# alberto-paparella/MusicRecommendation

Hardware: AMD Instinct MI355X
Metric: scored (test-user,song) pairs/sec, ItemBasedModel, 1/2/4/8 MI355X + mAP@10 (higher is better)
Workload: dtype int64

## Files before the change

### include/mr_engine.h

```cpp
#ifndef MR_ENGINE_H
#define MR_ENGINE_H

#include <stdint.h>
#include <stddef.h>

#ifdef __cplusplus
extern "C" {
#endif

#define MR_OK          0
#define MR_E_INVALID  -1
#define MR_E_HIP      -2
#define MR_E_OOM      -3
#define MR_E_STATE    -4
#define MR_E_IO       -5
#define MR_E_PARSE    -6
#define MR_E_RCCL     -7

#define MR_UBM 0
#define MR_IBM 1

#define MR_OUT_F32 0
#define MR_OUT_F64 1

// ... 42 lines not shown

int mr_launch_info(const mr_ctx* ctx, int32_t* shape, int32_t* block_songs, int32_t* n_tiles);

int mr_batch_info(const mr_ctx* ctx, int32_t* batch, int32_t* chunk, int32_t* n_chunks);

int mr_route_info(const mr_ctx* ctx, int32_t* route, int32_t* n_rows, int64_t* pool_entries);

int mr_topk_mode(const mr_ctx* ctx, int32_t* candidate_only);

int mr_cooc_stats(mr_ctx* ctx, int64_t* index_nnz, int64_t* consumed, int64_t* build_reads);

typedef struct mr_cooc_bytes_t {
  int64_t heavy_rows, light_rows;
  int64_t heavy_reads, light_reads;
  int64_t heavy_index_bytes, light_index_bytes;
  int64_t heavy_visits;
  int64_t consumed_bytes;
  int64_t group_tiles;
  int64_t n_groups;
  int64_t index_sparse_entries, index_dense_songs;
  int64_t consumed_sparse_entries, consumed_dense_songs;
} mr_cooc_bytes_t;
int mr_cooc_bytes(mr_ctx* ctx, mr_cooc_bytes_t* out);

int mr_shard_tile_songs(const mr_options* opt, int32_t n_train_users, int32_t n_test_users,
                        int32_t* tile_songs);

int mr_shard_tile_songs_n(const mr_options* opt, int32_t n_train_users, int32_t n_test_users, int32_t n_songs,
                          int32_t n_shards, int32_t* tile_songs);

int mr_run(mr_ctx* ctx, int model);
int mr_sync(mr_ctx* ctx);

int mr_graph_capture(mr_ctx* ctx, int model, int32_t n_steps);
int mr_graph_launch(mr_ctx* ctx);

int mr_device_outputs(const mr_ctx* ctx, void** dense, int32_t** topk_songs,
                      int64_t** topk_keys, double** topk_scores);

int mr_run_into(mr_ctx* ctx, int model, void* dense_dev);

typedef struct mr_view {
  int32_t n_test_users, n_songs, song_lo, song_hi, out_dtype, device;
  const int64_t* te_off;
  const int32_t* te_songs;
  void* stream;
// ... 134 lines not shown
```

### musicrecommendation_amd/_lib.py

```python
from __future__ import annotations

import ctypes
import os
from ctypes import POINTER, c_char_p, c_double, c_int, c_int32, c_int64, c_void_p

_HERE = os.path.dirname(os.path.abspath(__file__))
_VARIANT = os.environ.get("MR_ENGINE_LIB", "")
LIB_PATH = os.path.join(_HERE, f"libmr_engine_{_VARIANT}.so" if _VARIANT else "libmr_engine.so")

MR_OK = 0
MR_E_INVALID = -1
MR_E_HIP = -2
MR_E_OOM = -3
MR_E_STATE = -4
MR_E_IO = -5
MR_E_PARSE = -6
MR_E_RCCL = -7
MR_TRANSPORT_AUTO, MR_TRANSPORT_COPY, MR_TRANSPORT_RCCL = 0, 1, 2
MR_UBM = 0
MR_IBM = 1
STAGE1 = {"auto": 0, "fused": 1, "separate": 2, "wide": 4}
SHAPES = {0: "separate", 1: "fused", 3: "wide"}
MR_OUT_F32 = 0
MR_OUT_F64 = 1
# ... 80 lines not shown
MR_COMB_AGGREGATION = 1
MR_COMB_STOCHASTIC = 2
MR_SWEEP_MAX_PARAMS = 64


class EngineError(RuntimeError):
    def __init__(self, code: int, where: str, msg: str):
        super().__init__(f"{where}: {_ERRNAMES.get(code, code)}: {msg}")
        self.code = code


SIGNATURES = {
    "mr_options_default": (c_int, [POINTER(MrOptions)]),
    "mr_create": (c_int, [POINTER(MrOptions), POINTER(c_void_p)]),
    "mr_destroy": (c_int, [c_void_p]),
    "mr_load": (c_int, [c_void_p, POINTER(MrDataset)]),
    "mr_shard_info": (c_int, [c_void_p, POINTER(c_int32), POINTER(c_int32), POINTER(c_int32)]),
    "mr_launch_info": (c_int, [c_void_p, POINTER(c_int32), POINTER(c_int32), POINTER(c_int32)]),
    "mr_batch_info": (c_int, [c_void_p, POINTER(c_int32), POINTER(c_int32), POINTER(c_int32)]),
    "mr_route_info": (c_int, [c_void_p, POINTER(c_int32), POINTER(c_int32), POINTER(c_int64)]),
    "mr_topk_mode": (c_int, [c_void_p, POINTER(c_int32)]),
    "mr_cooc_stats": (c_int, [c_void_p, POINTER(c_int64), POINTER(c_int64), POINTER(c_int64)]),
    "mr_cooc_bytes": (c_int, [c_void_p, POINTER(MrCoocBytes)]),
    "mr_shard_tile_songs": (c_int, [POINTER(MrOptions), c_int32, c_int32, POINTER(c_int32)]),
    "mr_shard_tile_songs_n": (c_int, [POINTER(MrOptions), c_int32, c_int32, c_int32, c_int32, POINTER(c_int32)]),
    "mr_run": (c_int, [c_void_p, c_int]),
    "mr_sync": (c_int, [c_void_p]),
    "mr_graph_capture": (c_int, [c_void_p, c_int, c_int32]),
    "mr_graph_launch": (c_int, [c_void_p]),
    "mr_device_outputs": (c_int, [c_void_p, POINTER(c_void_p), POINTER(c_void_p), POINTER(c_void_p), POINTER(c_void_p)]),
    "mr_score_dense": (c_int, [c_void_p, c_int, c_void_p]),
    "mr_topk": (c_int, [c_void_p, c_int, c_int, c_void_p, c_void_p, c_void_p]),
    "mr_copy_dense": (c_int, [c_void_p, c_void_p]),
    "mr_copy_topk": (c_int, [c_void_p, c_void_p, c_void_p, c_void_p]),
    "mr_copy_topk_device": (c_int, [c_void_p, c_void_p, c_void_p]),
    "mr_copy_topk_device_async": (c_int, [c_void_p, c_void_p, c_void_p]),
    "mr_topk_merge_device_async": (c_int, [c_void_p, c_int32, c_int32, c_int32, c_void_p, c_void_p, c_void_p, c_void_p,
                                           c_void_p]),
    "mr_topk_record_bytes": (c_int, [c_int32, c_int32, POINTER(c_int64)]),
    "mr_topk_merge_records_async": (c_int, [c_void_p, c_int32, c_int32, c_int32, c_void_p, c_int64, c_void_p, c_void_p,
                                            c_void_p]),
    "mr_topk_merge_host": (c_int, [c_int32, c_int32, c_int32, c_void_p, c_void_p, c_void_p, c_void_p, c_void_p, c_void_p]),
    "mr_topk_merge_device": (c_int, [c_void_p, c_int32, c_int32, c_int32, c_void_p, c_void_p, c_void_p, c_void_p, c_void_p, c_void_p]),
    "mr_kernel_times": (c_int, [c_void_p, c_int32, POINTER(c_int64), POINTER(c_double), c_int32]),
    "mr_debug_stamps": (c_int, [c_void_p, c_void_p, c_int64]),
    "mr_timing_begin": (c_int, [c_void_p]),
# ... 93 lines not shown
```

### musicrecommendation_amd/csrc/mr_engine.hip

```cpp
#include <hip/hip_runtime.h>

#include <algorithm>
#include <atomic>
#include <climits>
#include <cmath>
#include <cstdarg>
#include <cstdio>
#include <cstdlib>
#include <cstring>
#include <limits>
#include <mutex>
#include <string>
#include <vector>

#ifndef MR_TILE_ROWS
#define MR_TILE_ROWS 32
#endif

#include "mr_engine.h"
#include "mr_internal.h"
#include "mr_par.h"


namespace {
// ... 2656 lines not shown
      run += wave_lane(inc, 63);
    }
    if (lane == 0) p.row_nnz[r] = (unsigned)run;
  }
  wave_lds_sync();
  stamp_rt_wave(sb, 3);
  unsigned* out = p.pool + p.row_base[r];
  for (int i = lane; i < S; i += 64) {
    const unsigned x = tab[i];
    if (x) {
      const int key = (int)((x >> kLightCntBits) - 1u);
      const int t = tile_of(key, bs, inv_bs);
      const int pos = atomicAdd(&tpos[t], 1);
      out[pos] = ((unsigned)(key - t * bs) << kCoocCntBits) | (x & kLightCntMask);
    }
  }
  wave_lds_sync();
  stamp_rt_wave(sb, 4);
  stamp_val(sb, 5, n, true);
  stamp_val(sb, 6, S, true);
  stamp_val(sb, 7, 64, true);
}

constexpr int kMaxGroupTiles = 8;
__host__ __device__ inline int cooc_group_lds(int bs, int g) {
  return align16(g * bs * 2) + 3 * kMaxGroupTiles * 4 + kMaxGroupTiles * 16 * 4;
}

__device__ __forceinline__ unsigned nz_halves(unsigned x) {
  return (((x & 0x7fff7fffu) + 0x7fff7fffu) | x) & 0x80008000u;
}
__device__ __forceinline__ int nz_pairs8(const uint4& w) {
  return __popc(nz_halves(w.x) | (nz_halves(w.y) >> 1) | (nz_halves(w.z) >> 2) | (nz_halves(w.w) >> 3));
}

template <int NT>
__device__ __forceinline__ void cooc_emit_group16(const CoocParams& p, int r, bool big, int t0, int ntg, int bs,
                                                  int width, const unsigned* cnt, int* s_wcnt, int* s_tail,
                                                  long long* off, unsigned* row_nz, long long* sb = nullptr) {
  constexpr int NW = NT / 64;
  const int tid = threadIdx.x, lane = tid & 63, w = tid >> 6;
  for (int k = 0; k < ntg; ++k) {
    const int bw = min(width, (t0 + k + 1) * bs) - (t0 + k) * bs;
    const uint4* cv = reinterpret_cast<const uint4*>(cnt + (size_t)k * (bs >> 1));
    const int nch = (bw + 7) >> 3;
    int nz = 0;
// ... 325 lines not shown
int light_tier_go(hipStream_t st, int n, const CoocParams* lp) {
  constexpr int NT = light_tier_nt(T), S = light_tier_slots(T);
  const int lds = cooc_light_lds<NT, S>();
  if (!lp) {
    MR_HIP(hipFuncSetAttribute((const void*)k_cooc_light<NT, S>, hipFuncAttributeMaxDynamicSharedMemorySize, lds));
    return MR_OK;
  }
  hipLaunchKernelGGL((k_cooc_light<NT, S>), dim3(n), dim3(NT), (size_t)lds, st, *lp);
  MR_HIP(hipGetLastError());
  return MR_OK;
}
template <int SW>
int light_wave_go(hipStream_t st, int n, const CoocParams* lp) {
  const int lds = cooc_wave_bytes<SW>() * kWaveRowsPerBlock;
  if (!lp) {
    MR_HIP(hipFuncSetAttribute((const void*)k_cooc_light_wave<SW>, hipFuncAttributeMaxDynamicSharedMemorySize, lds));
    return MR_OK;
  }
  hipLaunchKernelGGL(k_cooc_light_wave<SW>, dim3((n + kWaveRowsPerBlock - 1) / kWaveRowsPerBlock),
                     dim3(64 * kWaveRowsPerBlock), (size_t)lds, st, *lp, n);
  MR_HIP(hipGetLastError());
  return MR_OK;
}
int light_tier_call(int t, hipStream_t st, int n, const CoocParams* lp, const CoocParams&) {
  switch (t) {
    case 0: return light_tier_go<0>(st, n, lp);
    case 1: return light_tier_go<1>(st, n, lp);
    case 2: return light_tier_go<2>(st, n, lp);
    case 3: return light_tier_go<3>(st, n, lp);
    case 4: return light_wave_go<2048>(st, n, lp);
    default: return light_wave_go<1024>(st, n, lp);
  }
}

struct DenseTopkParams {
  int user0, width, song_lo, k;
  const void* dense;
  long long* top_key;
  int* top_song;
  double* top_score;
  unsigned* neg;
};

template <typename OutT>
__global__ __launch_bounds__(kWideThreads) void k_topk_dense(DenseTopkParams p) {
  constexpr int NT = kWideThreads, NW = NT / 64;
// ... 128 lines not shown
int dev_upload(DevBuf<T>& b, const T* src, size_t n, hipStream_t st) {
  int rc = dev_alloc(b, n);
  if (rc) return rc;
  if (n) MR_HIP(hipMemcpyAsync(b.p, src, n * sizeof(T), hipMemcpyHostToDevice, st));
  return MR_OK;
}

using ScoreKernel = void (*)(ScoreParams);
using NbrKernel = void (*)(NbrParams);

enum Shape { kShapeSeparate = 0, kShapeFused = 1, kShapeWide = 3 };

struct CoocPlan {
  int route = 1;
  std::vector<int32_t> row_song, te_row;
  std::vector<int64_t> row_base;
  std::vector<int64_t> row_reads;
  std::vector<int32_t> row_slots;
  std::vector<int32_t> heavy_rows, light_rows;
  std::vector<int32_t> shard_deg;
  std::vector<int32_t> row_users;
  std::vector<int32_t> row_listeners;
  std::vector<uint8_t> row_light;
  int64_t build_reads = 0;
  int64_t pool_cap = 0;
  int32_t max_shard_deg = 0;
  int n_light_tier[6] = {0, 0, 0, 0, 0, 0};
  bool all32 = false;
  int n_heavy32 = 0;
  int n_big16 = 0, tcap16 = 0, tcap32 = 0;
  int dense_div = 0, force32 = 0;
  unsigned sat = 255;
  int grp = 0, n_grp = 0, urec_words = 0, lrec_words = 0;
  int64_t n_lrec = 0;
  int64_t n_llrec = 0;
  int group_nt = 1024;
  int cooc_nt = 1024;
  int n_rows() const { return (int)row_song.size(); }
  int n_heavy() const { return (int)heavy_rows.size(); }
  int n_light() const { return (int)light_rows.size(); }
};

inline bool is_u32_row(const CoocPlan& p, int32_t listeners) { return p.all32 || listeners >= 65536; }

}

struct mr_ctx {
  mr_options opt{};
  int dev_share = 1;
  hipStream_t stream = nullptr;
  bool loaded = false;
  bool ran = false;
  bool fused = false;
  int shape = kShapeSeparate;
  int last_model = -1;
  int n_tr = 0, n_te = 0, n_s = 0;
  int song_lo = 0, song_hi = 0, width = 0;
  int block_songs = 0, n_tiles = 0;
  int cap = 0, batch = 0;
  int chunk = 1, n_chunks = 1;
  size_t score_lds = 0, nbr_lds = 0, merge_lds = 0, wide_lds = 0;
  ScoreKernel score_kernel[2] = {nullptr, nullptr};
  NbrKernel nbr_kernel[2] = {nullptr, nullptr};
// ... 30 lines not shown
  int graph_steps = 0;
  DevBuf<unsigned> flag;
  long long win_launches = 0;
  CoocPlan cooc;
  size_t cooc_score_lds = 0, cooc_lds = 0;
  int nseg = 0;
  ScoreKernel cooc_kernel = nullptr;
  DevBuf<int> row_song, te_row, seg_len;
  DevBuf<long long> row_base, seg_off;
  DevBuf<unsigned> pool;
  DevBuf<unsigned> row_nnz;
  bool cooc_ran = false;
  hipStream_t side[2] = {nullptr, nullptr};
  hipEvent_t side_fork = nullptr, side_join[2] = {nullptr, nullptr};
  size_t bstamp_off = 0;
  size_t lstamp_off = 0;
  DevBuf<int> rows_order, row_slots;
  DevBuf<int4> rdesc;
  DevBuf<long long> sr_off;
  DevBuf<unsigned> sr_songs;
  DevBuf<unsigned> urec;
  DevBuf<unsigned> lrec;
  DevBuf<uint2> llrec;

  void release_data() {
    tr_off.release(); te_off.release(); trs_off.release(); q_song.release();
    cand_key.release(); top_key.release(); nbr_q.release();
    tsongs.release(); tpack.release(); te_rng.release(); te_q.release(); te_sched.release(); sched_off.release(); te_songs.release(); trs_users.release(); toff.release(); sbound.release();
    nbr_v.release(); nbr_cnt.release(); cand_song.release(); top_song.release();
    counter.release();
    sqrt_c.release(); sqrt_tr.release(); sqrt_te.release(); top_score.release();
    rsq_c.release(); cand_on = false;
    dense.release();
    mm_key.release(); mm_on = mm_valid = false;
    stamps.release();
    flag.release();
    row_song.release(); te_row.release(); seg_len.release(); row_base.release(); seg_off.release();
    pool.release();
    rows_order.release(); row_slots.release(); sr_off.release(); sr_songs.release(); row_nnz.release();
    urec.release(); lrec.release(); llrec.release(); rdesc.release();
    cooc = CoocPlan{};
    cooc_kernel = nullptr;
    if (graph_exec) (void)hipGraphExecDestroy(graph_exec);
    if (graph) (void)hipGraphDestroy(graph);
    graph_exec = nullptr;
    graph = nullptr;
    graph_steps = 0;
    loaded = ran = cooc_ran = false;
// ... 59 lines not shown
    const int r = e ? std::atoi(e) : 32;
    return (r == 16 || r == 64) ? r : 32;
  }();
  return rows;
}

constexpr int64_t kLightSlotsNarrow = 8192;
int64_t cooc_light_max_opt(bool narrow) {
  const char* e = std::getenv("MR_COOC_LIGHT_MAX");
  int64_t v = e ? std::atoll(e) : (narrow ? kLightSlotsNarrow : kLightSlots);
  int64_t s = 1024;
  while (s * 2 <= std::min<int64_t>(v, kLightSlots)) s *= 2;
  return s;
}
int64_t cooc_light_load_opt() {
  const char* e = std::getenv("MR_COOC_LIGHT_LOAD");
  const int64_t v = e ? std::atoll(e) : 80;
  return std::min<int64_t>(100, std::max<int64_t>(10, v));
}
bool cooc_light_opt() {
  const char* e = std::getenv("MR_COOC_LIGHT");
  return !(e && std::atoi(e) == 0);
}
bool fused_sched_opt() {
  const char* e = std::getenv("MR_FUSED_SCHED");
  return MR_FUSED_SCHED && !(e && std::atoi(e) == 0);
}
int cooc_nt_opt() {
  const char* e = std::getenv("MR_COOC_NT");
  return e && std::atoi(e) == 512 ? 512 : 1024;
}
int cooc_group_nt_opt() {
  const char* e = std::getenv("MR_COOC_GNT");
  return e && std::atoi(e) == 512 ? 512 : 1024;
}
int cooc_group_max_opt() {
  const char* e = std::getenv("MR_COOC_GRP");
  const int v = e ? std::atoi(e) : 0;
  return v > 0 ? v : kMaxGroupTiles;
}
bool cooc_group_opt() {
  const char* e = std::getenv("MR_COOC_GROUP");
  return !(e && std::atoi(e) == 0);
}
bool cooc_side_opt() {
  const char* e = std::getenv("MR_COOC_SIDE");
  return !(e && std::atoi(e) == 0);
}
int cooc_dense_div_opt() {
  const char* e = std::getenv("MR_COOC_DENSE_DIV");
  return e ? std::max(0, std::atoi(e)) : kCoocDenseDiv;
}
int cooc_dense32_opt() {
  const char* e = std::getenv("MR_COOC_DENSE32");
  return e && std::atoi(e) == 1 ? 1 : 0;
}
unsigned cooc_sat_opt() {
  const char* e = std::getenv("MR_COOC_SAT");
  const long v = e ? std::atol(e) : 255;
  return (unsigned)std::min<long>(255, std::max<long>(1, v));
}

bool cooc_pays(double v_est, double e_est, const std::vector<int64_t>& bound, const std::vector<int64_t>& reads,
               const std::vector<int32_t>& row_song, const std::vector<int32_t>& col_tr, int n_tiles) {
  double build = 0.0;
  for (size_t r = 0; r < row_song.size(); ++r) {
    const double c = col_tr[row_song[r]];
    if (bound[r] <= light_bound_max(kLightSlots) && c <= kLightCntMask) build += 12.8e-12 * (double)(reads[r] - c) + 28e-9;
    else build += n_tiles * (35e-12 * c + 24e-9);
  }
  return build + 0.49e-12 * e_est < 5.75e-12 * v_est;
}

int wide_map_opt() {
  static const int m = [] {
    const char* e = std::getenv("MR_WIDE_MAP");
    const int v = e ? std::atoi(e) : 0;
    return v >= 1 && v <= 3 ? v : kWideMapDefault;
  }();
  return m;
}

int auto_block_songs(int width, int n_te, bool fused, int k, int n_tr) {
  long long cover = ((long long)width + 255) / 256 * 256;
  if (!fused && n_tr > kMaxLdsTrainUsers && k <= kMaxTopkLarge)
    return (int)std::max<long long>(256, std::min<long long>(kMaxBlockSongs, cover));
  const long long cap = k > 0 ? kMaxTopkTile : (fused ? 8192 : kMaxBlockSongs);
  const long long target = fused ? 256 : 1024;
  long long want = ((long long)width * std::max(1, n_te) + target - 1) / target;
  long long bs = ((want + 255) / 256) * 256;
  bs = std::max<long long>(256, std::min<long long>(cap, bs));
  return (int)std::max<long long>(256, std::min(bs, cover));
// ... 387 lines not shown
      return "a cheaper estimate than the two-hop route (auto)";
  }
  return nullptr;
}

void cooc_split(const CoocIn& in, CoocPlan& p) {
  const std::vector<int32_t>& col_tr = in.col_tr;
  const int width = in.lp.width, n_tiles = in.lp.n_tiles, bs = in.lp.block_songs;
  const int64_t nr = p.n_rows();
  const bool light_ok = width <= kLightMaxWidth && n_tiles <= kLightMaxTiles && cooc_light_opt();
  bool narrow = false;
  if (cooc_group_opt() && 1 + (n_tiles + 2) / 2 <= 32 && p.max_shard_deg <= 65535 &&
      n_tiles <= std::min(kMaxGroupTiles, cooc_group_max_opt()))
    narrow = cooc_group_lds(bs, n_tiles) <= kLdsBytes;
  const int64_t lload = cooc_light_load_opt(), light_slots_max = cooc_light_max_opt(narrow);
  p.dense_div = cooc_dense_div_opt();
  int64_t dense_pad = 0;
  for (int t = 0; t < n_tiles; ++t) {
    const int bw = (int)(std::min<int64_t>(width, (int64_t)(t + 1) * bs) - (int64_t)t * bs);
    dense_pad += cooc_dense_words(bw) - (bw + 3) / 4;
  }
  dense_pad = (dense_pad + 3) & ~(int64_t)3;
  p.row_slots.assign((size_t)std::max<int64_t>(1, nr), 0);
  for (int64_t r = 0; r < nr; ++r) {
    const int64_t c = col_tr[p.row_song[r]];
    if (light_ok && p.row_base[r] * 100 <= light_slots_max * lload && c <= (int32_t)kLightCntMask) {
      int sl = 1024;
      while ((int64_t)sl * lload < p.row_base[r] * 100) sl <<= 1;
      p.row_slots[r] = sl | (walk_glog(c > 0 ? (p.row_reads[r] - c) / c : 0) << kLightGlogShift);
      p.light_rows.push_back((int32_t)r);
      p.row_base[r] = (p.row_base[r] + 3) & ~(int64_t)3;
    } else {
      const int64_t nz = p.row_base[r];
      const int64_t dn = std::max<int64_t>(1, std::min<int64_t>(p.dense_div, width)) * nz;
      p.row_base[r] = ((std::min<int64_t>(width, dn) + nz + 3) & ~(int64_t)3) + 8 * (int64_t)n_tiles + dense_pad;
      p.heavy_rows.push_back((int32_t)r);
    }
  }
  std::vector<int32_t>& heavy_rows = p.heavy_rows;
  p.force32 = cooc_dense32_opt();
  p.all32 = !MR_COOC_P16 || p.force32;
  std::stable_partition(heavy_rows.begin(), heavy_rows.end(),
                        [&](int32_t r) { return is_u32_row(p, col_tr[p.row_song[r]]); });
  for (int32_t r : heavy_rows) p.n_heavy32 += is_u32_row(p, col_tr[p.row_song[r]]) ? 1 : 0;
  const int sparse_max = p.dense_div > 0 ? (bs + p.dense_div - 1) / p.dense_div : bs;
  p.tcap32 = (std::max(sparse_max, cooc_dense_words(bs) + bs) + 7) & ~7;
  p.tcap16 = p.tcap32;
  for (size_t i = p.n_heavy32; i < heavy_rows.size(); ++i) {
    if (col_tr[p.row_song[heavy_rows[i]]] < kCoocBigRow) break;
// ... 20 lines not shown
      if ((int)i >= p.n_heavy32 + p.n_big16)
        while (glog > 0 && cr > (int64_t)(p.group_nt >> glog) * kGroupPipeR) --glog;
      p.row_slots[r] = glog << kLightGlogShift;
    }
  } else {
    p.urec_words = 0;
  }
  p.pool_cap = mr_par::exclusive_scan(p.row_base.data(), nr);
  p.row_base[nr] = p.pool_cap;
}

void cooc_records(const CoocIn& in, CoocPlan& p) {
  if (p.grp > 0) {
    for (size_t i = p.n_heavy32; i < p.heavy_rows.size(); ++i) p.n_lrec += in.col_tr[p.row_song[p.heavy_rows[i]]];
    p.lrec_words = 1;
    while (2 * (p.lrec_words - 1) < p.n_grp + 1) p.lrec_words <<= 1;
  }
  for (int32_t r : p.light_rows) p.n_llrec += in.col_tr[p.row_song[r]];
}

void cooc_finish(const CoocIn& in, CoocPlan& p) {
  const int n_tiles = in.lp.n_tiles;
  const auto tier = [&](int32_t r) { return light_tier(p.row_slots[r] & kLightSlotsMask, n_tiles); };
  std::stable_sort(p.light_rows.begin(), p.light_rows.end(), [&](int32_t x, int32_t y) { return tier(x) < tier(y); });
  for (int32_t r : p.light_rows) p.n_light_tier[tier(r)]++;
  const size_t nr = p.row_song.size();
  for (int64_t x : p.row_reads) p.build_reads += x;
  p.row_users.assign(nr, 0);
  for (size_t i = 0; i < (size_t)in.d->te_off[in.d->n_test_users]; ++i)
    if (p.te_row[i] >= 0) p.row_users[p.te_row[i]]++;
  p.row_listeners.resize(nr);
  for (size_t r = 0; r < nr; ++r) p.row_listeners[r] = in.col_tr[p.row_song[r]];
  p.row_light.assign(nr, 0);
  for (int32_t r : p.light_rows) p.row_light[r] = 1;
  p.sat = cooc_sat_opt();
  p.cooc_nt = cooc_nt_opt();
  p.route = 2;
}

int plan_cooc(const CoocIn& in, size_t free_b, int dev_share, CoocPlan* out, const char** why) {
  *out = CoocPlan{};
  *why = nullptr;
  if (!in.lp.wide()) *why = "the wide shape only";
  else if (in.lp.block_songs > kCoocMaxTile) *why = "song tiles <= 32768";
  if (in.opt.ibm_route == 1) return MR_OK;
  CoocPlan p;
  if (!*why) *why = cooc_rows(in, p);
  if (!*why) *why = cooc_bounds(in, p);
  if (!*why) {
    cooc_split(in, p);
    for (int64_t r = 0; r < p.n_rows(); ++r)
      if (p.row_base[r] & 3)
        return fail(MR_E_STATE, "co-listening index: row %lld starts at word %lld (not 16-B aligned)",
                    (long long)r, (long long)p.row_base[r]);
    cooc_records(in, p);
// ... 96 lines not shown
  if ((rc = dev_alloc(c->pool, (size_t)p.pool_cap))) return rc;
  const size_t n_heavy = p.heavy_rows.size();
  std::vector<int32_t> order(p.heavy_rows);
  order.insert(order.end(), p.light_rows.begin(), p.light_rows.end());
  if ((rc = dev_upload(c->rows_order, order.data(), order.size(), st))) return rc;
  {
    std::vector<int4> rd(std::max<size_t>(1, order.size()));
    int64_t at_lrec = 0, at_llrec = 0;
    for (size_t i = 0; i < order.size(); ++i) {
      const int32_t r = order[i], s2 = p.row_song[r];
      const int cnt = (int)(trs_off[s2 + 1] - trs_off[s2]);
      int z = (int)trs_off[s2];
      if (p.grp > 0 && (int)i >= p.n_heavy32 && i < n_heavy) {
        z = (int)at_lrec;
        at_lrec += cnt;
      } else if (i >= n_heavy) {
        z = (int)at_llrec;
        at_llrec += cnt;
      }
      rd[i] = make_int4(r, p.row_slots[r], z, cnt);
    }
    if ((rc = dev_upload(c->rdesc, rd.data(), rd.size(), st))) return rc;
    MR_HIP(hipStreamSynchronize(st));
  }
  if ((rc = dev_upload(c->row_slots, p.row_slots.data(), p.row_slots.size(), st))) return rc;
  if (p.light_rows.empty() && p.grp == 0) return MR_OK;
  std::vector<int64_t> so((size_t)n_tr + 1, 0);
  std::copy(p.shard_deg.begin(), p.shard_deg.begin() + n_tr, so.begin());
  so[n_tr] = mr_par::exclusive_scan(so.data(), (int64_t)n_tr);
  mr_par::buffer<uint32_t> ss((size_t)so[n_tr] + 4);
  std::fill(ss.begin() + so[n_tr], ss.end(), 0u);
  mr_par::parallel_for(n_tr, [&](int64_t a, int64_t b, int) {
    for (int64_t v = a; v < b; ++v) {
      const int32_t* r0 = std::lower_bound(ti.songs.data() + ti.off[v], ti.songs.data() + ti.off[v + 1], lo);
      for (int64_t i = 0; i < so[v + 1] - so[v]; ++i) ss[so[v] + i] = (uint32_t)(r0[i] - lo);
    }
  });
  if ((rc = dev_upload(c->sr_off, reinterpret_cast<const long long*>(so.data()), so.size(), st))) return rc;
  if ((rc = dev_upload(c->sr_songs, ss.data(), ss.size(), st))) return rc;
  if (!p.light_rows.empty()) {
    if ((rc = dev_alloc(c->llrec, (size_t)std::max<int64_t>(1, p.n_llrec)))) return rc;
    hipLaunchKernelGGL(k_llrec, dim3((unsigned)p.light_rows.size()), dim3(256), 0, st, c->rdesc.p + n_heavy,
                       c->row_song.p, c->trs_off.p, c->trs_users.p, c->sr_off.p, c->llrec.p);
    MR_HIP(hipGetLastError());
  }
  if (p.grp > 0) {
    if ((rc = dev_alloc(c->urec, (size_t)std::max(1, n_tr) * p.urec_words))) return rc;
    hipLaunchKernelGGL(k_urec, dim3((std::max(1, n_tr) + 255) / 256), dim3(256), 0, st, c->sr_off.p,
                       c->sr_songs.p, n_tr, n_tiles, lp.block_songs, p.urec_words, c->urec.p);
    MR_HIP(hipGetLastError());
    if ((rc = dev_alloc(c->lrec, (size_t)std::max<int64_t>(1, p.n_lrec) * p.lrec_words))) return rc;
    const int n16 = (int)n_heavy - p.n_heavy32;
    if (n16 > 0)
      hipLaunchKernelGGL(k_lrec, dim3(n16), dim3(256), 0, st, c->rdesc.p + p.n_heavy32, c->row_song.p,
                         c->trs_off.p, c->trs_users.p, c->urec.p, p.urec_words, n_tiles, p.grp, p.n_grp, p.lrec_words,
                         c->lrec.p);
    MR_HIP(hipGetLastError());
    MR_HIP(hipStreamSynchronize(st));
    c->urec.release();
  }
  MR_HIP(hipStreamSynchronize(st));
  return MR_OK;
}

int alloc_outputs(mr_ctx* c, const LaunchPlan& lp, int route, int n_te) {
  hipStream_t st = c->stream;
  const int k = lp.k;
// ... 48 lines not shown
    const WideLds<kWideThreads> WL = p.cooc_nt == 512 ? wide_lds<512>(bs, k, n_chunks).as_wide()
                                                      : wide_lds<kWideThreads>(bs, k, n_chunks);
    c->cooc_score_lds = (size_t)WL.total;
    c->nseg = std::min(std::min(p.cooc_nt, (WL.total - WL.wk - 8) / 40), 255);
    if (c->nseg < 16) return fail(MR_E_INVALID, "co-listening route: no LDS for row descriptors");
    c->cooc_lds = (size_t)cooc_build_lds<false>(bs);
    if (p.grp > 0)
      MR_HIP(hipFuncSetAttribute(p.group_nt == 512 ? (const void*)k_cooc_group<512> : (const void*)k_cooc_group<1024>,
                                 hipFuncAttributeMaxDynamicSharedMemorySize, cooc_group_lds(bs, p.grp)));
    for (int t = 0; t < kLightTiers; ++t)
      if (int rc2 = light_tier_call(t, nullptr, 0, nullptr, CoocParams{})) return rc2;
    MR_HIP(hipFuncSetAttribute((const void*)c->cooc_kernel, hipFuncAttributeMaxDynamicSharedMemorySize,
                               (int)c->cooc_score_lds));
    MR_HIP(hipFuncSetAttribute((const void*)k_cooc_build<MR_COOC_NT, false>, hipFuncAttributeMaxDynamicSharedMemorySize,
                               (int)c->cooc_lds));
    MR_HIP(hipFuncSetAttribute((const void*)k_cooc_build<MR_COOC_NT16, true>, hipFuncAttributeMaxDynamicSharedMemorySize,
                               cooc_build_lds<true>(bs)));
  }
  if (wide && k > 0) {
    c->merge_lds = (size_t)merge_lds_bytes(k);
    MR_HIP(hipFuncSetAttribute((const void*)k_topk_merge, hipFuncAttributeMaxDynamicSharedMemorySize,
                               (int)c->merge_lds));
  }
  return MR_OK;
}

}


extern "C" {

const char* mr_last_error(void) { return g_err.c_str(); }
const char* mr_version(void) { return "mr_engine 0.2 (gfx950)"; }

int mr_options_default(mr_options* opt) {
  if (!opt) return fail(MR_E_INVALID, "null options");
  std::memset(opt, 0, sizeof *opt);
  opt->device = 0;
  opt->frac_bits = 32;
  opt->song_lo = 0;
  opt->song_hi = 0;
  opt->block_songs = 0;
  opt->out_dtype = MR_OUT_F32;
  opt->topk = 10;
  opt->dense = 1;
  opt->time_kernels = 0;
// ... 155 lines not shown
  if (!c->loaded) return fail(MR_E_STATE, "mr_route_info before mr_load");
  if (route) *route = c->cooc.route;
  if (n_rows) *n_rows = c->cooc.n_rows();
  if (pool_entries) *pool_entries = c->cooc.pool_cap;
  return MR_OK;
}

int mr_topk_mode(const mr_ctx* c, int32_t* candidate_only) {
  if (!c || !candidate_only) return fail(MR_E_INVALID, "null argument");
  if (!c->loaded) return fail(MR_E_STATE, "mr_topk_mode before mr_load");
  *candidate_only = c->cand_on ? 1 : 0;
  return MR_OK;
}

int mr_cooc_stats(mr_ctx* c, int64_t* index_nnz, int64_t* consumed, int64_t* build_reads) {
  if (!c) return fail(MR_E_INVALID, "null context");
  if (!c->loaded || c->cooc.route != 2) return fail(MR_E_STATE, "mr_cooc_stats needs a context on ibm_route 2");
  if (!c->cooc_ran) return fail(MR_E_STATE, "mr_cooc_stats before an ibm run");
  MR_HIP(hipSetDevice(c->opt.device));
  std::vector<unsigned> nnz((size_t)std::max(1, c->cooc.n_rows()), 0u);
  if (c->cooc.n_rows() > 0)
    MR_HIP(hipMemcpyAsync(nnz.data(), c->row_nnz.p, (size_t)c->cooc.n_rows() * 4, hipMemcpyDeviceToHost, c->stream));
  MR_HIP(hipStreamSynchronize(c->stream));
  int64_t tot = 0, use = 0;
  for (int r = 0; r < c->cooc.n_rows(); ++r) {
    tot += nnz[r];
    use += (int64_t)nnz[r] * c->cooc.row_users[r];
  }
  if (index_nnz) *index_nnz = tot;
  if (consumed) *consumed = use;
  if (build_reads) *build_reads = c->cooc.build_reads;
  return MR_OK;
}

int mr_cooc_bytes(mr_ctx* c, mr_cooc_bytes_t* out) {
  if (!c || !out) return fail(MR_E_INVALID, "null argument");
  if (!c->loaded || c->cooc.route != 2) return fail(MR_E_STATE, "mr_cooc_bytes needs a context on ibm_route 2");
  if (!c->cooc_ran) return fail(MR_E_STATE, "mr_cooc_bytes before an ibm run");
  MR_HIP(hipSetDevice(c->opt.device));
  const CoocPlan& p = c->cooc;
  const int nr = p.n_rows(), nt = c->n_tiles;
  std::vector<int32_t> len((size_t)std::max(1, nr) * nt, 0);
  if (nr > 0)
    MR_HIP(hipMemcpyAsync(len.data(), c->seg_len.p, (size_t)nr * nt * 4, hipMemcpyDeviceToHost, c->stream));
  MR_HIP(hipStreamSynchronize(c->stream));
  mr_cooc_bytes_t b{};
  for (int r = 0; r < nr; ++r) {
    int64_t seg = 0;
    int64_t sp = 0, ds = 0;
    for (int t = 0; t < nt; ++t) {
      const int blo = c->song_lo + t * c->block_songs;
      const int64_t bw = std::min(c->song_hi, blo + c->block_songs) - blo;
      const int32_t l = len[(size_t)t * nr + r];
      seg += l >= 0 ? std::min<int64_t>(4 * (int64_t)l, bw) : bw;
      if (l >= 0) sp += l;
      else { ds += bw; sp += kCoocDenseTail - l; }
    }
    b.index_sparse_entries += sp;
    b.index_dense_songs += ds;
    b.consumed_sparse_entries += sp * p.row_users[r];
    b.consumed_dense_songs += ds * p.row_users[r];
    if (p.row_light[r]) {
      b.light_rows++;
      b.light_reads += p.row_reads[r];
      b.light_index_bytes += seg;
    } else {
      b.heavy_rows++;
      b.heavy_reads += p.row_reads[r];
      b.heavy_index_bytes += seg;
      const bool u32row = is_u32_row(c->cooc, p.row_listeners[r]);
      b.heavy_visits += (int64_t)p.row_listeners[r] * (p.grp > 0 && !u32row ? p.n_grp : nt);
    }
    b.consumed_bytes += seg * p.row_users[r];
  }
  b.group_tiles = p.grp;
  b.n_groups = p.grp > 0 ? p.n_grp : nt;
  *out = b;
  return MR_OK;
}

int mr_shard_info(const mr_ctx* c, int32_t* lo, int32_t* hi, int32_t* n_te) {
  if (!c) return fail(MR_E_INVALID, "null context");
  if (!c->loaded) return fail(MR_E_STATE, "mr_shard_info before mr_load");
  if (lo) *lo = c->song_lo;
  if (hi) *hi = c->song_hi;
  if (n_te) *n_te = c->n_te;
  return MR_OK;
}

int mr_launch_info(const mr_ctx* c, int32_t* fused, int32_t* block_songs, int32_t* n_tiles) {
  if (!c) return fail(MR_E_INVALID, "null context");
  if (!c->loaded) return fail(MR_E_STATE, "mr_launch_info before mr_load");
  if (fused) *fused = c->shape;
  if (block_songs) *block_songs = c->block_songs;
  if (n_tiles) *n_tiles = c->n_tiles;
  return MR_OK;
}

int mr_batch_info(const mr_ctx* c, int32_t* batch, int32_t* chunk, int32_t* n_chunks) {
  if (!c) return fail(MR_E_INVALID, "null context");
// ... 94 lines not shown
      hp.grp = p.grp;
      hp.n_grp = p.n_grp;
      hp.rdesc = c->rdesc.p + n32;
      if (hp.stamps) hp.stamps += (size_t)n32 * c->n_tiles * 8;
      const int nblk = (p.n_big16 + 7) / 8 * 8 * p.n_grp + (n16 - p.n_big16);
      const size_t glds = (size_t)cooc_group_lds(c->block_songs, p.grp);
      if (p.group_nt == 512)
        hipLaunchKernelGGL(k_cooc_group<512>, dim3(nblk), dim3(512), glds, st, hp);
      else
        hipLaunchKernelGGL(k_cooc_group<1024>, dim3(nblk), dim3(1024), glds, st, hp);
      MR_HIP(hipGetLastError());
    } else if (n16 > 0) {
      CoocParams hp = cp;
      hp.rows = c->rows_order.p + n32;
      hp.n_big = p.n_big16;
      hp.tcap = p.tcap16;
      if (hp.stamps) hp.stamps += (size_t)n32 * c->n_tiles * 8;
      hipLaunchKernelGGL((k_cooc_build<MR_COOC_NT16, true>), dim3(p.n_big16 * c->n_tiles + n16 - p.n_big16),
                         dim3(MR_COOC_NT16),
                         (size_t)cooc_build_lds<true>(c->block_songs), st, hp);
      MR_HIP(hipGetLastError());
    }
    int lr = p.n_heavy();
    for (int t = 0; t < kLightTiers; ++t) {
      if (p.n_light_tier[t] == 0) continue;
      CoocParams lp = cp;
      lp.rows = c->rows_order.p + lr;
      lp.rdesc = c->rdesc.p + lr;
      lp.llrec = reinterpret_cast<const unsigned*>(c->llrec.p);
      lp.lstamps = c->stamps.p ? c->stamps.p + c->lstamp_off + (size_t)(lr - p.n_heavy()) * 8 : nullptr;
      hipStream_t ls = side ? c->side[t < 2 ? 0 : 1] : st;
      if (int rc2 = light_tier_call(t, ls, p.n_light_tier[t], &lp, lp)) return rc2;
      lr += p.n_light_tier[t];
    }
    if (side)
      for (int i = 0; i < 2; ++i) {
        MR_HIP(hipEventRecord(c->side_join[i], c->side[i]));
        MR_HIP(hipStreamWaitEvent(st, c->side_join[i], 0));
      }
  }
  if (timed) MR_HIP(hipEventRecord(ev[1], st));
  for (int y0 = 0; y0 < c->n_te; y0 += 65528) {
    const int ny = std::min(65528, c->n_te - y0);
    const int remap = wide_map_opt();
    ScoreParams sp{};
    sp.chunk = c->chunk; sp.n_chunks = c->n_chunks;
// ... 561 lines not shown
```

### musicrecommendation_amd/engine.py

```python
from __future__ import annotations

import ctypes
from typing import Optional, Tuple, Union

import numpy as np

from . import _lib
from .dataset import Dataset

MODELS = {"ubm": _lib.MR_UBM, "ibm": _lib.MR_IBM, _lib.MR_UBM: _lib.MR_UBM, _lib.MR_IBM: _lib.MR_IBM}
KERNELS = {"neighbours": 0, "score": 1}
IBM_ROUTES = {"auto": 0, "two_hop": 1, "cooc": 2}


def model_id(model: Union[str, int]) -> int:
    try:
        return MODELS[model]
    except KeyError:
        raise ValueError(f"unknown model {model!r}: use 'ubm' or 'ibm'") from None


class Engine:
    def __init__(self, dataset: Dataset, *, device: int = 0, frac_bits: int = 32, song_lo: int = 0,
                 song_hi: int = 0, block_songs: int = 0, out_dtype: str = "f32", topk: int = 10,
# ... 62 lines not shown

    def __exit__(self, *exc):
        self.close()

    def __del__(self):
        try:
            self.close()
        except Exception:
            pass

    def run(self, model: Union[str, int]) -> None:
        _lib.check(self._L.mr_run(self._h, model_id(model)), "mr_run")

    def cooc_stats(self) -> Tuple[int, int, int]:
        a, b, c = ctypes.c_int64(), ctypes.c_int64(), ctypes.c_int64()
        _lib.check(self._L.mr_cooc_stats(self._h, ctypes.byref(a), ctypes.byref(b), ctypes.byref(c)), "mr_cooc_stats")
        return a.value, b.value, c.value

    def cooc_bytes(self) -> dict:
        b = _lib.MrCoocBytes()
        _lib.check(self._L.mr_cooc_bytes(self._h, ctypes.byref(b)), "mr_cooc_bytes")
        return {name: int(getattr(b, name)) for name, _t in _lib.MrCoocBytes._fields_}

    def sync(self) -> None:
        _lib.check(self._L.mr_sync(self._h), "mr_sync")

    def graph_capture(self, model: Union[str, int], n_steps: int) -> None:
        _lib.check(self._L.mr_graph_capture(self._h, model_id(model), int(n_steps)), "mr_graph_capture")

    def graph_launch(self) -> None:
        _lib.check(self._L.mr_graph_launch(self._h), "mr_graph_launch")

    @property
    def stream(self) -> int:
        return self._L.mr_stream(self._h) or 0

    def dense(self) -> np.ndarray:
        out = np.empty((self.n_test, self.width), dtype=self.dtype)
        _lib.check(self._L.mr_copy_dense(self._h, out.ctypes.data_as(ctypes.c_void_p)), "mr_copy_dense")
        return out

    def topk(self) -> Tuple[np.ndarray, np.ndarray, np.ndarray]:
        k = self.topk_k
        songs = np.empty((self.n_test, k), dtype=np.int32)
        scores = np.empty((self.n_test, k), dtype=np.float64)
        keys = np.empty((self.n_test, k), dtype=np.int64)
# ... 220 lines not shown
```

Before: 16.95 billion.

## Add list-mode light co-occurrence rows that emit raw entries without dedup

Adds a new k_cooc_list kernel for light rows whose co-occurrence entry count is small. It writes each co-song entry straight into per-tile segments with count 1, instead of aggregating through the light hash tables. A one-time COUNT pass at setup precomputes segment offsets and lengths, so the per-run pass only scatters. The cost model and row partitioning are updated to route such rows to this path, split between workgroup and wavefront launches. The trade-off is duplicate entries left in the pool for the consumer to handle, plus host-side stats reconstruction for diagnostics.

```diff
diff --git a/include/mr_engine.h b/include/mr_engine.h
--- a/include/mr_engine.h
+++ b/include/mr_engine.h
@@ -88,6 +88,8 @@
   int64_t consumed_sparse_entries, consumed_dense_songs;
 } mr_cooc_bytes_t;
 int mr_cooc_bytes(mr_ctx* ctx, mr_cooc_bytes_t* out);
+
+int mr_cooc_list_info(const mr_ctx* ctx, int64_t* list_rows, int64_t* list_entries);
 
 int mr_shard_tile_songs(const mr_options* opt, int32_t n_train_users, int32_t n_test_users,
                         int32_t* tile_songs);
diff --git a/musicrecommendation_amd/_lib.py b/musicrecommendation_amd/_lib.py
--- a/musicrecommendation_amd/_lib.py
+++ b/musicrecommendation_amd/_lib.py
@@ -126,6 +126,7 @@
     "mr_topk_mode": (c_int, [c_void_p, POINTER(c_int32)]),
     "mr_cooc_stats": (c_int, [c_void_p, POINTER(c_int64), POINTER(c_int64), POINTER(c_int64)]),
     "mr_cooc_bytes": (c_int, [c_void_p, POINTER(MrCoocBytes)]),
+    "mr_cooc_list_info": (c_int, [c_void_p, POINTER(c_int64), POINTER(c_int64)]),
     "mr_shard_tile_songs": (c_int, [POINTER(MrOptions), c_int32, c_int32, POINTER(c_int32)]),
     "mr_shard_tile_songs_n": (c_int, [POINTER(MrOptions), c_int32, c_int32, c_int32, c_int32, POINTER(c_int32)]),
     "mr_run": (c_int, [c_void_p, c_int]),
diff --git a/musicrecommendation_amd/csrc/mr_engine.hip b/musicrecommendation_amd/csrc/mr_engine.hip
--- a/musicrecommendation_amd/csrc/mr_engine.hip
+++ b/musicrecommendation_amd/csrc/mr_engine.hip
@@ -2702,6 +2702,71 @@
   stamp_val(sb, 7, 64, true);
 }
 
+constexpr int kListWgThreads = 256;
+template <int NT, bool COUNT>
+__global__ __launch_bounds__(NT) void k_cooc_list(CoocParams p) {
+  extern __shared__ __align__(16) unsigned char smem_raw[];
+  int* tpos = reinterpret_cast<int*>(smem_raw);
+  const int4 rd = p.rdesc[blockIdx.x];
+  const int r = rd.x;
+  const int tid = threadIdx.x;
+  long long* sb = p.lstamps ? p.lstamps + (size_t)blockIdx.x * 8 : nullptr;
+  stamp_rt(sb, 0);
+  const long long base = p.row_base[r];
+  for (int t = tid; t < p.n_tiles; t += NT)
+    tpos[t] = COUNT ? 0 : (int)(p.seg_off[(size_t)t * p.n_rows + r] - base);
+  const int n = rd.w;
+  const unsigned* lst = p.llrec + 2 * (size_t)(unsigned)rd.z;
+  __syncthreads();
+  stamp_rt(sb, 1);
+  const int bs = p.block_songs;
+  const float inv_bs = 1.0f / (float)bs;
+  unsigned* out = p.pool + base;
+  rows_walk(tid, NT, rd.y >> kLightGlogShift, [](int l) { return l; }, n, ShardRow{lst}, p.sr_songs,
+            [&](const unsigned (&k)[8], int m) {
+              int tl[8];
+#pragma unroll
+              for (int i = 0; i < 8; ++i) tl[i] = i < m ? tile_of((int)k[i], bs, inv_bs) : -1 - i;
+              int pos = 0;
+#pragma unroll
+              for (int i = 0; i < 8; ++i) {
+                if (i < m) {
+                  if (i == 0 || tl[i] != tl[i - 1]) {
+                    int len = 0;
+#pragma unroll
+                    for (int j = i; j < 8; ++j) len += tl[j] == tl[i] ? 1 : 0;
+                    pos = atomicAdd(&tpos[tl[i]], len);
+                  }
+                  if (!COUNT) out[pos] = ((unsigned)((int)k[i] - tl[i] * bs) << kCoocCntBits) | 1u;
+                  ++pos;
+                }
+              }
+            });
+  if constexpr (COUNT) {
+    __syncthreads();
+    if (tid < 64) {
+      int run = 0;
+      for (int t0 = 0; t0 < p.n_tiles; t0 += 64) {
+        const int t = t0 + tid;
+        const int c = t < p.n_tiles ? tpos[t] : 0;
+        const int inc = wave_incl_scan(c);
+        if (t < p.n_tiles) {
+          p.seg_off[(size_t)t * p.n_rows + r] = base + run + inc - c;
+          p.seg_len[(size_t)t * p.n_rows + r] = c;
+        }
+        run += wave_lane(inc, 63);
+      }
+    }
+  } else {
+    stamp_rt(sb, 2);
+    stamp_rt(sb, 3);
+    stamp_rt(sb, 4);
+    stamp_val(sb, 5, n);
+    stamp_val(sb, 6, 1);
+    stamp_val(sb, 7, NT);
+  }
+}
+
 constexpr int kMaxGroupTiles = 8;
 __host__ __device__ inline int cooc_group_lds(int bs, int g) {
   return align16(g * bs * 2) + 3 * kMaxGroupTiles * 4 + kMaxGroupTiles * 16 * 4;
@@ -3073,6 +3138,22 @@
   MR_HIP(hipGetLastError());
   return MR_OK;
 }
+template <bool COUNT>
+int list_rows_go(hipStream_t st_wg, hipStream_t st_wave, int n_wg, int n_wave, const CoocParams& lp) {
+  const size_t lds = (size_t)align16(lp.n_tiles * 4);
+  if (n_wg > 0) {
+    hipLaunchKernelGGL((k_cooc_list<kListWgThreads, COUNT>), dim3(n_wg), dim3(kListWgThreads), lds, st_wg, lp);
+    MR_HIP(hipGetLastError());
+  }
+  if (n_wave > 0) {
+    CoocParams wp = lp;
+    wp.rdesc += n_wg;
+    if (wp.lstamps) wp.lstamps += (size_t)n_wg * 8;
+    hipLaunchKernelGGL((k_cooc_list<64, COUNT>), dim3(n_wave), dim3(64), lds, st_wave, wp);
+    MR_HIP(hipGetLastError());
+  }
+  return MR_OK;
+}
 int light_tier_call(int t, hipStream_t st, int n, const CoocParams* lp, const CoocParams&) {
   switch (t) {
     case 0: return light_tier_go<0>(st, n, lp);
@@ -3247,6 +3328,9 @@
   std::vector<int32_t> row_users;
   std::vector<int32_t> row_listeners;
   std::vector<uint8_t> row_light;
+  std::vector<uint8_t> row_list;
+  int n_list_wg = 0, n_list_wave = 0;
+  int64_t list_entries = 0;
   int64_t build_reads = 0;
   int64_t pool_cap = 0;
   int32_t max_shard_deg = 0;
@@ -3264,6 +3348,7 @@
   int n_rows() const { return (int)row_song.size(); }
   int n_heavy() const { return (int)heavy_rows.size(); }
   int n_light() const { return (int)light_rows.size(); }
+  int n_list() const { return n_list_wg + n_list_wave; }
 };
 
 inline bool is_u32_row(const CoocPlan& p, int32_t listeners) { return p.all32 || listeners >= 65536; }
@@ -3340,8 +3425,13 @@
   DevBuf<unsigned> urec;
   DevBuf<unsigned> lrec;
   DevBuf<uint2> llrec;
+  std::vector<int4> list_rd;
+  std::vector<int32_t> list_len;
+  std::vector<unsigned> list_nnz;
+  bool list_stats = false;
 
   void release_data() {
+    list_rd.clear(); list_len.clear(); list_nnz.clear(); list_stats = false;
     tr_off.release(); te_off.release(); trs_off.release(); q_song.release();
     cand_key.release(); top_key.release(); nbr_q.release();
     tsongs.release(); tpack.release(); te_rng.release(); te_q.release(); te_sched.release(); sched_off.release(); te_songs.release(); trs_users.release(); toff.release(); sbound.release();
@@ -3447,6 +3537,20 @@
   const char* e = std::getenv("MR_COOC_LIGHT");
   return !(e && std::atoi(e) == 0);
 }
+bool cooc_list_opt() {
+  const char* e = std::getenv("MR_COOC_LIST");
+  return !(e && std::atoi(e) == 0);
+}
+int64_t cooc_list_users_opt() {
+  const char* e = std::getenv("MR_COOC_LIST_USERS");
+  const int64_t v = e ? std::atoll(e) : 0;
+  return v > 0 ? v : INT64_MAX;
+}
+int64_t cooc_list_wg_opt() {
+  const char* e = std::getenv("MR_COOC_LIST_WG");
+  const int64_t v = e ? std::atoll(e) : 0;
+  return v > 0 ? v : 4096;
+}
 bool fused_sched_opt() {
   const char* e = std::getenv("MR_FUSED_SCHED");
   return MR_FUSED_SCHED && !(e && std::atoi(e) == 0);
@@ -3489,10 +3593,16 @@
 bool cooc_pays(double v_est, double e_est, const std::vector<int64_t>& bound, const std::vector<int64_t>& reads,
                const std::vector<int32_t>& row_song, const std::vector<int32_t>& col_tr, int n_tiles) {
   double build = 0.0;
+  const bool list = cooc_light_opt() && cooc_list_opt();
   for (size_t r = 0; r < row_song.size(); ++r) {
     const double c = col_tr[row_song[r]];
-    if (bound[r] <= light_bound_max(kLightSlots) && c <= kLightCntMask) build += 12.8e-12 * (double)(reads[r] - c) + 28e-9;
-    else build += n_tiles * (35e-12 * c + 24e-9);
+    const double occ = (double)(reads[r] - c);
+    if (bound[r] <= light_bound_max(kLightSlots) && c <= kLightCntMask) {
+      if (list && (double)bound[r] == occ) build += 1.1e-12 * occ + 35e-9;
+      else build += 12.8e-12 * occ + 28e-9;
+    } else {
+      build += n_tiles * (35e-12 * c + 24e-9);
+    }
   }
   return build + 0.49e-12 * e_est < 5.75e-12 * v_est;
 }
@@ -3926,9 +4036,18 @@
   }
   dense_pad = (dense_pad + 3) & ~(int64_t)3;
   p.row_slots.assign((size_t)std::max<int64_t>(1, nr), 0);
+  p.row_users.assign((size_t)nr, 0);
+  for (size_t i = 0; i < (size_t)in.d->te_off[in.d->n_test_users]; ++i)
+    if (p.te_row[i] >= 0) p.row_users[p.te_row[i]]++;
+  p.row_list.assign((size_t)std::max<int64_t>(1, nr), 0);
+  const bool list_on = cooc_light_opt() && cooc_list_opt();
+  const int64_t list_users = cooc_list_users_opt();
   for (int64_t r = 0; r < nr; ++r) {
     const int64_t c = col_tr[p.row_song[r]];
-    if (light_ok && p.row_base[r] * 100 <= light_slots_max * lload && c <= (int32_t)kLightCntMask) {
+    const int64_t occ = p.row_reads[r] - c;
+    const bool fits = p.row_base[r] * 100 <= light_slots_max * lload && c <= (int32_t)kLightCntMask;
+    p.row_list[r] = fits && list_on && occ <= width && occ < 32768 && p.row_users[r] <= list_users;
+    if (fits && (light_ok || p.row_list[r])) {
       int sl = 1024;
       while ((int64_t)sl * lload < p.row_base[r] * 100) sl <<= 1;
       p.row_slots[r] = sl | (walk_glog(c > 0 ? (p.row_reads[r] - c) / c : 0) << kLightGlogShift);
@@ -3995,15 +4114,21 @@
 void cooc_finish(const CoocIn& in, CoocPlan& p) {
   const int n_tiles = in.lp.n_tiles;
   const auto tier = [&](int32_t r) { return light_tier(p.row_slots[r] & kLightSlotsMask, n_tiles); };
-  std::stable_sort(p.light_rows.begin(), p.light_rows.end(), [&](int32_t x, int32_t y) { return tier(x) < tier(y); });
-  for (int32_t r : p.light_rows) p.n_light_tier[tier(r)]++;
   const size_t nr = p.row_song.size();
   for (int64_t x : p.row_reads) p.build_reads += x;
-  p.row_users.assign(nr, 0);
-  for (size_t i = 0; i < (size_t)in.d->te_off[in.d->n_test_users]; ++i)
-    if (p.te_row[i] >= 0) p.row_users[p.te_row[i]]++;
   p.row_listeners.resize(nr);
   for (size_t r = 0; r < nr; ++r) p.row_listeners[r] = in.col_tr[p.row_song[r]];
+  const auto occ = [&](int32_t r) { return p.row_reads[r] - p.row_listeners[r]; };
+  const int64_t list_wg = cooc_list_wg_opt();
+  const auto list_end = std::stable_partition(p.light_rows.begin(), p.light_rows.end(),
+                                              [&](int32_t r) { return p.row_list[r] != 0; });
+  std::stable_sort(p.light_rows.begin(), list_end, [&](int32_t x, int32_t y) { return occ(x) > occ(y); });
+  for (auto it = p.light_rows.begin(); it != list_end; ++it) {
+    (occ(*it) >= list_wg ? p.n_list_wg : p.n_list_wave)++;
+    p.list_entries += occ(*it);
+  }
+  std::stable_sort(list_end, p.light_rows.end(), [&](int32_t x, int32_t y) { return tier(x) < tier(y); });
+  for (auto it = list_end; it != p.light_rows.end(); ++it) p.n_light_tier[tier(*it)]++;
   p.row_light.assign(nr, 0);
   for (int32_t r : p.light_rows) p.row_light[r] = 1;
   p.sat = cooc_sat_opt();
@@ -4146,6 +4271,7 @@
     }
     if ((rc = dev_upload(c->rdesc, rd.data(), rd.size(), st))) return rc;
     MR_HIP(hipStreamSynchronize(st));
+    c->list_rd.assign(rd.begin() + n_heavy, rd.begin() + n_heavy + p.n_list());
   }
   if ((rc = dev_upload(c->row_slots, p.row_slots.data(), p.row_slots.size(), st))) return rc;
   if (p.light_rows.empty() && p.grp == 0) return MR_OK;
@@ -4167,6 +4293,20 @@
     hipLaunchKernelGGL(k_llrec, dim3((unsigned)p.light_rows.size()), dim3(256), 0, st, c->rdesc.p + n_heavy,
                        c->row_song.p, c->trs_off.p, c->trs_users.p, c->sr_off.p, c->llrec.p);
     MR_HIP(hipGetLastError());
+  }
+  if (p.n_list() > 0) {
+    CoocParams cp{};
+    cp.n_rows = (int)nr;
+    cp.n_tiles = n_tiles;
+    cp.block_songs = lp.block_songs;
+    cp.row_base = c->row_base.p;
+    cp.pool = c->pool.p;
+    cp.seg_off = c->seg_off.p;
+    cp.seg_len = c->seg_len.p;
+    cp.sr_songs = c->sr_songs.p;
+    cp.llrec = reinterpret_cast<const unsigned*>(c->llrec.p);
+    cp.rdesc = c->rdesc.p + n_heavy;
+    if ((rc = list_rows_go<true>(st, st, p.n_list_wg, p.n_list_wave, cp))) return rc;
   }
   if (p.grp > 0) {
     if ((rc = dev_alloc(c->urec, (size_t)std::max(1, n_tr) * p.urec_words))) return rc;
@@ -4261,6 +4401,90 @@
     MR_HIP(hipFuncSetAttribute((const void*)k_topk_merge, hipFuncAttributeMaxDynamicSharedMemorySize,
                                (int)c->merge_lds));
   }
+  return MR_OK;
+}
+
+int ensure_list_stats(mr_ctx* c) {
+  const CoocPlan& p = c->cooc;
+  const int nl = p.n_list(), nt = c->n_tiles, nr = p.n_rows();
+  if (c->list_stats || nl == 0) return MR_OK;
+  hipStream_t st = c->stream;
+  if (c->width > kLightMaxWidth || nt > kLightMaxTiles) {
+    std::vector<long long> off((size_t)nr * nt);
+    std::vector<int32_t> len((size_t)nr * nt);
+    MR_HIP(hipMemcpyAsync(off.data(), c->seg_off.p, off.size() * 8, hipMemcpyDeviceToHost, st));
+    MR_HIP(hipMemcpyAsync(len.data(), c->seg_len.p, len.size() * 4, hipMemcpyDeviceToHost, st));
+    MR_HIP(hipStreamSynchronize(st));
+    c->list_len.assign((size_t)nl * nt, 0);
+    c->list_nnz.assign((size_t)nl, 0u);
+    std::vector<unsigned> buf;
+    for (int i = 0; i < nl; ++i) {
+      const int r = c->list_rd[i].x;
+      const size_t n = (size_t)(p.row_reads[r] - p.row_listeners[r]);
+      buf.resize(std::max<size_t>(1, n));
+      if (n) MR_HIP(hipMemcpy(buf.data(), c->pool.p + p.row_base[r], n * 4, hipMemcpyDeviceToHost));
+      for (int t = 0; t < nt; ++t) {
+        unsigned* a = buf.data() + (off[(size_t)t * nr + r] - p.row_base[r]);
+        unsigned* b = a + len[(size_t)t * nr + r];
+        std::sort(a, b);
+        const int32_t d = (int32_t)(std::unique(a, b) - a);
+        c->list_len[(size_t)i * nt + t] = d;
+        c->list_nnz[i] += (unsigned)d;
+      }
+    }
+    c->list_stats = true;
+    return MR_OK;
+  }
+  const auto tier = [&](int i) { return light_tier(c->list_rd[i].y & kLightSlotsMask, nt); };
+  std::vector<int> idx(nl);
+  for (int i = 0; i < nl; ++i) idx[i] = i;
+  std::stable_sort(idx.begin(), idx.end(), [&](int x, int y) { return tier(x) < tier(y); });
+  std::vector<int4> rd(nl);
+  int n_tier[kLightTiers] = {};
+  for (int i = 0; i < nl; ++i) {
+    rd[i] = c->list_rd[idx[i]];
+    n_tier[tier(idx[i])]++;
+  }
+  struct Scratch {
+    DevBuf<int4> rd;
+    DevBuf<int> len;
+    DevBuf<long long> off;
+    DevBuf<unsigned> nnz;
+    ~Scratch() { rd.release(); len.release(); off.release(); nnz.release(); }
+  } s;
+  int rc;
+  if ((rc = dev_upload(s.rd, rd.data(), rd.size(), st))) return rc;
+  if ((rc = dev_alloc(s.len, (size_t)nr * nt))) return rc;
+  if ((rc = dev_alloc(s.off, (size_t)nr * nt))) return rc;
+  if ((rc = dev_alloc(s.nnz, (size_t)nr))) return rc;
+  CoocParams cp{};
+  cp.n_tr = c->n_tr; cp.n_rows = nr; cp.n_tiles = nt; cp.block_songs = c->block_songs;
+  cp.song_lo = c->song_lo; cp.song_hi = c->song_hi;
+  cp.row_song = c->row_song.p; cp.row_base = c->row_base.p; cp.pool = c->pool.p;
+  cp.seg_off = s.off.p; cp.seg_len = s.len.p; cp.row_nnz = s.nnz.p;
+  cp.sr_off = c->sr_off.p; cp.sr_songs = c->sr_songs.p; cp.row_slots = c->row_slots.p;
+  cp.llrec = reinterpret_cast<const unsigned*>(c->llrec.p);
+  int at = 0;
+  for (int t = 0; t < kLightTiers; ++t) {
+    if (n_tier[t] == 0) continue;
+    CoocParams lp = cp;
+    lp.rdesc = s.rd.p + at;
+    if ((rc = light_tier_call(t, st, n_tier[t], &lp, lp))) return rc;
+    at += n_tier[t];
+  }
+  std::vector<int32_t> len((size_t)nr * nt);
+  std::vector<unsigned> nnz((size_t)nr);
+  MR_HIP(hipMemcpyAsync(len.data(), s.len.p, len.size() * 4, hipMemcpyDeviceToHost, st));
+  MR_HIP(hipMemcpyAsync(nnz.data(), s.nnz.p, nnz.size() * 4, hipMemcpyDeviceToHost, st));
+  MR_HIP(hipStreamSynchronize(st));
+  c->list_len.assign((size_t)nl * nt, 0);
+  c->list_nnz.assign((size_t)nl, 0u);
+  for (int i = 0; i < nl; ++i) {
+    const int r = c->list_rd[i].x;
+    c->list_nnz[i] = nnz[r];
+    for (int t = 0; t < nt; ++t) c->list_len[(size_t)i * nt + t] = len[(size_t)t * nr + r];
+  }
+  c->list_stats = true;
   return MR_OK;
 }
 
@@ -4462,6 +4686,8 @@
   if (c->cooc.n_rows() > 0)
     MR_HIP(hipMemcpyAsync(nnz.data(), c->row_nnz.p, (size_t)c->cooc.n_rows() * 4, hipMemcpyDeviceToHost, c->stream));
   MR_HIP(hipStreamSynchronize(c->stream));
+  if (int rc = ensure_list_stats(c)) return rc;
+  for (size_t i = 0; i < c->list_nnz.size(); ++i) nnz[c->list_rd[i].x] = c->list_nnz[i];
   int64_t tot = 0, use = 0;
   for (int r = 0; r < c->cooc.n_rows(); ++r) {
     tot += nnz[r];
@@ -4484,6 +4710,9 @@
   if (nr > 0)
     MR_HIP(hipMemcpyAsync(len.data(), c->seg_len.p, (size_t)nr * nt * 4, hipMemcpyDeviceToHost, c->stream));
   MR_HIP(hipStreamSynchronize(c->stream));
+  if (int rc = ensure_list_stats(c)) return rc;
+  for (size_t i = 0; i < c->list_nnz.size(); ++i)
+    for (int t = 0; t < nt; ++t) len[(size_t)t * nr + c->list_rd[i].x] = c->list_len[i * nt + t];
   mr_cooc_bytes_t b{};
   for (int r = 0; r < nr; ++r) {
     int64_t seg = 0;
@@ -4516,6 +4745,14 @@
   b.group_tiles = p.grp;
   b.n_groups = p.grp > 0 ? p.n_grp : nt;
   *out = b;
+  return MR_OK;
+}
+
+int mr_cooc_list_info(const mr_ctx* c, int64_t* list_rows, int64_t* list_entries) {
+  if (!c) return fail(MR_E_INVALID, "null context");
+  if (!c->loaded || c->cooc.route != 2) return fail(MR_E_STATE, "mr_cooc_list_info needs a context on ibm_route 2");
+  if (list_rows) *list_rows = c->cooc.n_list();
+  if (list_entries) *list_entries = c->cooc.list_entries;
   return MR_OK;
 }
 
@@ -4656,6 +4893,15 @@
       MR_HIP(hipGetLastError());
     }
     int lr = p.n_heavy();
+    if (p.n_list() > 0) {
+      CoocParams lp = cp;
+      lp.rdesc = c->rdesc.p + lr;
+      lp.llrec = reinterpret_cast<const unsigned*>(c->llrec.p);
+      lp.lstamps = c->stamps.p ? c->stamps.p + c->lstamp_off : nullptr;
+      if (int rc2 = list_rows_go<false>(side ? c->side[0] : st, side ? c->side[1] : st, p.n_list_wg, p.n_list_wave, lp))
+        return rc2;
+      lr += p.n_list();
+    }
     for (int t = 0; t < kLightTiers; ++t) {
       if (p.n_light_tier[t] == 0) continue;
       CoocParams lp = cp;
diff --git a/musicrecommendation_amd/engine.py b/musicrecommendation_amd/engine.py
--- a/musicrecommendation_amd/engine.py
+++ b/musicrecommendation_amd/engine.py
@@ -108,6 +108,11 @@
         _lib.check(self._L.mr_cooc_bytes(self._h, ctypes.byref(b)), "mr_cooc_bytes")
         return {name: int(getattr(b, name)) for name, _t in _lib.MrCoocBytes._fields_}
 
+    def cooc_list_info(self) -> Tuple[int, int]:
+        a, b = ctypes.c_int64(), ctypes.c_int64()
+        _lib.check(self._L.mr_cooc_list_info(self._h, ctypes.byref(a), ctypes.byref(b)), "mr_cooc_list_info")
+        return a.value, b.value
+
     def sync(self) -> None:
         _lib.check(self._L.mr_sync(self._h), "mr_sync")
 
```

Result: no change. 16.97 billion, median of 4 (+0.1%).
